# Eclectic-Sheep/sheeprl

Measured on NVIDIA H100. Metric: Dreamer-V3 train-steps/sec (S, bs16 seq64 horizon15, 64x64x3 obs), higher is better.
Workload: dtype f32

## Files before the change

sheeprl_b200/csrc/gemm_tc.cu:

```cuda
#include <cuda.h>
#include <cudaTypedefs.h>

#include <mutex>
#include <unordered_map>

#include "common.cuh"

namespace {

constexpr int BM = 128, BK = 32;
constexpr int NTHREADS = 384;
constexpr int NSPLIT_THREADS = 96;
constexpr int NCONS_WARPS = 8;
constexpr int PRODUCER_REGS = 56, CONSUMER_REGS = 224;
template <int BN> constexpr int stages_for() { return BN == 128 ? 3 : 5; }

__device__ __forceinline__ uint32_t smem_u32(const void* p) { return (uint32_t)__cvta_generic_to_shared(p); }

__device__ __forceinline__ void mbar_init(uint64_t* bar, uint32_t count) {
  asm volatile("mbarrier.init.shared::cta.b64 [%0], %1;" ::"r"(smem_u32(bar)), "r"(count) : "memory");
}
__device__ __forceinline__ void mbar_expect_tx(uint64_t* bar, uint32_t bytes) {
  asm volatile("mbarrier.arrive.expect_tx.shared::cta.b64 _, [%0], %1;" ::"r"(smem_u32(bar)), "r"(bytes) : "memory");
}
// ... 577 lines not shown
      c[j] = r;
    }
  }
}

#define LAUNCH_GEMM_TC(BN_, PASSES_, grid_, st_, ...)                                                                \
  do {                                                                                                               \
    const size_t smem__ = sizeof(Smem<BN_>) + 1024;                                                                  \
    RL_CUDA(cudaFuncSetAttribute(gemm_tc_kernel<BN_, PASSES_>, cudaFuncAttributeMaxDynamicSharedMemorySize, (int)smem__)); \
    gemm_tc_kernel<BN_, PASSES_><<<grid_, NTHREADS, smem__, st_>>>(__VA_ARGS__);                                      \
  } while (0)
#define DISPATCH_GEMM_TC(BN_val, passes_val, grid_, st_, ...)                                  \
  do {                                                                                          \
    if ((BN_val) == 64) {                                                                       \
      if ((passes_val) == 3) LAUNCH_GEMM_TC(64, 3, grid_, st_, __VA_ARGS__);                    \
      else LAUNCH_GEMM_TC(64, 1, grid_, st_, __VA_ARGS__);                                      \
    } else {                                                                                    \
      if ((passes_val) == 3) LAUNCH_GEMM_TC(128, 3, grid_, st_, __VA_ARGS__);                   \
      else LAUNCH_GEMM_TC(128, 1, grid_, st_, __VA_ARGS__);                                     \
    }                                                                                           \
  } while (0)

int launch_conv(int mode, const float* img, const float* Wp, float* out, const float* bias, int NB, int h, int w, int Cin,
                int Cout, cudaStream_t st) {
  TileGeo g = {};
  g.mode = mode; g.h = h; g.w = w; g.NB = NB; g.chunks = Cin / BK; g.Cout = Cout; g.ksplits = 1;
  g.passes = g_passes;
  RL_CHECK_ARG(conv_tile(h, w, NB, &g.bw, &g.bh, &g.bn), "image grid not tileable by 128 pixels");
  g.tiles_x = w / g.bw; g.tiles_y = h / g.bh;
  if (mode == MODE_UP && conv_up_merged(Cout)) mode = g.mode = MODE_UP4;
  const int taps = mode == MODE_DOWN ? 16 : (mode == MODE_UP4 ? 9 : 4);
  const int K = taps * Cin;
  CUtensorMap ma, mb;
  if (mode == MODE_DOWN) { if (int rc = get_map4(img, Cin, 2 * w, 2 * h, NB, g.bw, g.bh, g.bn, 2, &ma)) return rc; }
  else                   { if (int rc = get_map4(img, Cin, w, h, NB, g.bw, g.bh, g.bn, 1, &ma)) return rc; }
  const int BN = (mode == MODE_UP4) ? 128 : ((Cout <= 64) ? 64 : 128);
  const int brows = (mode == MODE_UP || mode == MODE_UP4) ? 4 * Cout : Cout;
  if (int rc = get_map(Wp, brows, K, K, BN, &mb)) return rc;
  const int mtiles = g.tiles_x * g.tiles_y * (NB / g.bn);
  g.mtiles = mtiles;
  g.ntiles = (mode == MODE_UP4) ? 1 : (Cout + BN - 1) / BN;
  dim3 grid(1, 1, mode == MODE_UP ? 4 : 1);
  grid.y = persistent_grid_y(mtiles * g.ntiles, grid.z);
  const int M = NB * h * w;
  DISPATCH_GEMM_TC(BN, g.passes, grid, st, ma, mb, out, bias, M, Cout, K, Cout, 0, g);
  RL_CHECK_LAUNCH();
  return B200RL_OK;
}

}

extern "C" int b200rl_set_matmul_precision(int tf32_passes) {
  RL_CHECK_ARG(tf32_passes == 1 || tf32_passes == 3, "tf32_passes must be 3 (fp32-accurate 3xTF32) or 1 (single TF32 pass)");
  g_passes = tf32_passes;
  return B200RL_OK;
}
extern "C" int b200rl_get_matmul_precision(void) { return g_passes; }

extern "C" long long b200rl_conv_pack_floats(int mode_up, int Cs, int Cb) {
  return (mode_up && conv_up_merged(Cb) ? 36LL : 16LL) * Cs * Cb;
}
extern "C" int b200rl_conv_tc_supported(int mode_up, int NB, int h, int w, int Cs, int Cb) {
  int bw, bh, bn;
  if (!conv_tile(h, w, NB, &bw, &bh, &bn)) return 0;
  const int Cin = mode_up ? Cs : Cb, Cout = mode_up ? Cb : Cs;
  if (Cin % BK != 0 || Cout < 16 || Cout % 4 != 0) return 0;
  return 1;
}
extern "C" int b200rl_conv_pack(const float* W, float* Wpacked, int mode_up, int Cs, int Cb, cudaStream_t st) {
  RL_CHECK_ARG(W && Wpacked, "null pointer");
  const long long n = (long long)Cs * Cb * 16;
  if (mode_up && conv_up_merged(Cb)) conv_pack_up4_kernel<<<ceil_div(36LL * Cs * Cb, 256), 256, 0, st>>>(W, Wpacked, Cs, Cb);
  else if (mode_up) conv_pack_up_kernel<<<ceil_div(n, 256), 256, 0, st>>>(W, Wpacked, Cs, Cb);
  else conv_pack_down_kernel<<<ceil_div(n, 256), 256, 0, st>>>(W, Wpacked, Cs, Cb);
  RL_CHECK_LAUNCH();
  return B200RL_OK;
}
extern "C" int b200rl_conv_down_tc(const float* big, const float* Wpacked, float* small_, int NB, int h, int w, int Cs,
                                   int Cb, cudaStream_t st) {
  RL_CHECK_ARG(big && Wpacked && small_, "null pointer");
  RL_CHECK_ARG(b200rl_conv_tc_supported(0, NB, h, w, Cs, Cb), "shape not eligible for the tensor-core conv path");
  return launch_conv(MODE_DOWN, big, Wpacked, small_, nullptr, NB, h, w, Cb, Cs, st);
}
extern "C" int b200rl_conv_up_tc(const float* small_, const float* Wpacked, float* big, const float* bias, int NB, int h,
                                 int w, int Cs, int Cb, cudaStream_t st) {
  RL_CHECK_ARG(big && Wpacked && small_, "null pointer");
  RL_CHECK_ARG(b200rl_conv_tc_supported(1, NB, h, w, Cs, Cb), "shape not eligible for the tensor-core conv path");
  return launch_conv(MODE_UP, small_, Wpacked, big, bias, NB, h, w, Cs, Cb, st);
}

extern "C" int b200rl_gemm_tc_supported(const float* A, const float* B, int M, int N, int K, int lda, int ldb,
                                        int transA, int transB) {
  (void)transA; (void)transB;
  if (M < 32 || N < 48 || K < 32) return 0;
  if ((lda & 3) || (ldb & 3)) return 0;
  if ((reinterpret_cast<uintptr_t>(A) & 15) || (reinterpret_cast<uintptr_t>(B) & 15)) return 0;
  return 1;
}

namespace {
struct FusedTail { float* part; int ks, mpad, ldw; };

int gemm_tc_impl(const float* A, const float* B, float* C, const float* bias, int M, int N, int K, int lda,
                 int ldb, int ldc, int transA, int transB, int accumulate, cudaStream_t st, FusedTail* fused) {
  RL_CHECK_ARG(A && B && (C || fused), "null pointer");
  RL_CHECK_ARG(b200rl_gemm_tc_supported(A, B, M, N, K, lda, ldb, transA, transB), "shape not eligible for the tensor-core path");
  const int BN = (N <= 64) ? 64 : 128;
  CUtensorMap ma, mb;
  if (!transA) { if (int rc = get_map(A, M, K, lda, BM, &ma)) return rc; }
  else         { if (int rc = get_map(A, K, M, lda, 32, &ma)) return rc; }
  if (transB)  { if (int rc = get_map(B, N, K, ldb, BN, &mb)) return rc; }
  else         { if (int rc = get_map(B, K, N, ldb, 32, &mb)) return rc; }
  dim3 grid((N + BN - 1) / BN, (M + BM - 1) / BM);
  TileGeo g = {};
  g.mode = MODE_GEMM;
  g.a_mn = transA ? 1 : 0;
  g.b_mn = transB ? 0 : 1;
  g.ksplits = 1;
  g.passes = g_passes;
  const int tiles = grid.x * grid.y, nkb = (K + BK - 1) / BK;
  if (tiles < 2 * kNumSMs && nkb >= 8) {
    int best = 1;
    float best_t = 1e30f;
    const int max_sp = nkb / 4 < 32 ? nkb / 4 : 32;
    for (int sp = 1; sp <= (max_sp < 1 ? 1 : max_sp); ++sp) {
      const int per = (nkb + sp - 1) / sp, real = (nkb + per - 1) / per;
      const int waves = (tiles * real + kNumSMs - 1) / kNumSMs;
      const float t = waves * (per * 0.8f + 4.0f) + (real > 1 ? 3.0f + 0.3f * real : 0.0f);
      if (t < best_t - 1e-3f) { best_t = t; best = real; }
    }
    g.ksplits = best;
  }
  if (g.ksplits > 1 || fused) {
    grid.z = g.ksplits;
    g.mpad = (int)grid.y * BM;
    g.ldw = (int)grid.x * BN;
    if (int rc = split_workspace((size_t)g.ksplits * g.mpad * g.ldw, st, &g.part)) return rc;
    if (fused) { g.force_part = 1; *fused = FusedTail{g.part, g.ksplits, g.mpad, g.ldw}; }
  }
  g.mtiles = (int)grid.y;
  g.ntiles = (int)grid.x;
  grid.x = 1;
  grid.y = persistent_grid_y(g.mtiles * g.ntiles, grid.z);
  DISPATCH_GEMM_TC(BN, g.passes, grid, st, ma, mb, C, bias, M, N, K, ldc, accumulate, g);
  RL_CHECK_LAUNCH();
  if (g.ksplits > 1 && !fused) {
    splitk_reduce_kernel<<<ceil_div((long long)M * ((N + 3) / 4), 256), 256, 0, st>>>(g.part, C, bias, M, N, ldc, g.ksplits, g.mpad,
                                                                                      g.ldw, accumulate);
    RL_CHECK_LAUNCH();
  }
  return B200RL_OK;
}

template <int NV>
__global__ void __launch_bounds__(256)
splitk_ln_kernel(const float* __restrict__ part, int ks, int mpad, int ldw, int M, int N, const float* __restrict__ gamma,
                 const float* __restrict__ beta, float eps, int act, float* __restrict__ pre, long long ldpre,
                 float* __restrict__ ln_out, long long ldln, int mode, const float* __restrict__ h_prev, long long ldh,
                 float* __restrict__ h_out, long long ldho, float* __restrict__ h_out2, long long ldho2) {
  const int lane = threadIdx.x & 31;
  const long long row = ((long long)blockIdx.x * blockDim.x + threadIdx.x) >> 5;
  if (row >= M) return;
  const int n4 = N >> 2;
  float4 v[NV];
#pragma unroll
  for (int i = 0; i < NV; ++i) v[i] = make_float4(0.f, 0.f, 0.f, 0.f);
#pragma unroll 4
  for (int z = 0; z < ks; ++z) {
    const float4* p = reinterpret_cast<const float4*>(part + ((size_t)z * mpad + row) * ldw);
#pragma unroll
    for (int i = 0; i < NV; ++i) {
      const int c = lane + 32 * i;
      if (c < n4) { const float4 t = __ldcg(p + c); v[i].x += t.x; v[i].y += t.y; v[i].z += t.z; v[i].w += t.w; }
    }
  }
  float s = 0.f;
#pragma unroll
  for (int i = 0; i < NV; ++i) {
    const int c = lane + 32 * i;
    if (c < n4) {
      if (pre) reinterpret_cast<float4*>(pre + row * ldpre)[c] = v[i];
      s += (v[i].x + v[i].y) + (v[i].z + v[i].w);
    }
  }
  const float mu = warp_sum(s) / (float)N;
  float q = 0.f;
#pragma unroll
  for (int i = 0; i < NV; ++i) {
    const int c = lane + 32 * i;
    if (c < n4) {
      const float dx = v[i].x - mu, dy = v[i].y - mu, dz = v[i].z - mu, dw = v[i].w - mu;
      q += (dx * dx + dy * dy) + (dz * dz + dw * dw);
    }
  }
  const float rstd = rsqrtf(warp_sum(q) / (float)N + eps);
#pragma unroll
  for (int i = 0; i < NV; ++i) {
    const int c = lane + 32 * i;
    if (c < n4) {
      const float4 g = reinterpret_cast<const float4*>(gamma)[c], b = reinterpret_cast<const float4*>(beta)[c];
      v[i].x = (v[i].x - mu) * rstd * g.x + b.x; v[i].y = (v[i].y - mu) * rstd * g.y + b.y;
      v[i].z = (v[i].z - mu) * rstd * g.z + b.z; v[i].w = (v[i].w - mu) * rstd * g.w + b.w;
      if (mode == 0 && act == 1) {
        v[i].x = v[i].x / (1.f + expf(-v[i].x)); v[i].y = v[i].y / (1.f + expf(-v[i].y));
        v[i].z = v[i].z / (1.f + expf(-v[i].z)); v[i].w = v[i].w / (1.f + expf(-v[i].w));
      }
      if (ln_out) reinterpret_cast<float4*>(ln_out + row * ldln)[c] = v[i];
    }
  }
  if (mode == 1) {
    constexpr int NR = NV / 3;
#pragma unroll
    for (int i = 0; i < NR; ++i) {
      const int c = lane + 32 * i;
      const float4 hp = reinterpret_cast<const float4*>(h_prev + row * ldh)[c];
      const float4 gr = v[i], gc = v[i + NR], gu = v[i + 2 * NR];
      float4 h;
      auto gate = [](float r_, float c_, float u_, float hprev) {
        const float r = 1.f / (1.f + expf(-r_));
        const float cand = tanhf(r * c_);
        const float u = 1.f / (1.f + expf(-(u_ - 1.f)));
        return u * cand + (1.f - u) * hprev;
      };
      h.x = gate(gr.x, gc.x, gu.x, hp.x); h.y = gate(gr.y, gc.y, gu.y, hp.y);
      h.z = gate(gr.z, gc.z, gu.z, hp.z); h.w = gate(gr.w, gc.w, gu.w, hp.w);
      reinterpret_cast<float4*>(h_out + row * ldho)[c] = h;
      if (h_out2) reinterpret_cast<float4*>(h_out2 + row * ldho2)[c] = h;
    }
  }
}
}

extern "C" int b200rl_gemm_tc(const float* A, const float* B, float* C, const float* bias, int M, int N, int K, int lda,
                              int ldb, int ldc, int transA, int transB, int accumulate, cudaStream_t st) {
  return gemm_tc_impl(A, B, C, bias, M, N, K, lda, ldb, ldc, transA, transB, accumulate, st, nullptr);
}

extern "C" int b200rl_gemm_ln_supported(const float* A, const float* B, int M, int N, int K, int lda, int ldb, int mode) {
  if (!b200rl_gemm_tc_supported(A, B, M, N, K, lda, ldb, 0, 1)) return 0;
  if (N % 4 || N > 1536) return 0;
  if (mode == 1 && (N % 384 != 0)) return 0;
  return 1;
}

extern "C" int b200rl_gemm_ln(const float* A, const float* W, int M, int N, int K, int lda, int ldw_, const float* gamma,
                              const float* beta, float eps, int act, float* pre, long long ldpre, float* out, long long ldout,
                              int mode, const float* h_prev, long long ldh, float* h_out, long long ldho, float* h_out2,
                              long long ldho2, cudaStream_t st) {
  RL_CHECK_ARG(A && W && gamma && beta, "null pointer");
  RL_CHECK_ARG(b200rl_gemm_ln_supported(A, W, M, N, K, lda, ldw_, mode), "shape not eligible for the fused product + LayerNorm");
  RL_CHECK_ARG(mode == 0 ? out != nullptr : (h_prev && h_out), "missing output");
  RL_CHECK_ARG(((reinterpret_cast<uintptr_t>(gamma) | reinterpret_cast<uintptr_t>(beta) | reinterpret_cast<uintptr_t>(pre) |
                 reinterpret_cast<uintptr_t>(out) | reinterpret_cast<uintptr_t>(h_prev) | reinterpret_cast<uintptr_t>(h_out) |
                 reinterpret_cast<uintptr_t>(h_out2)) & 15) == 0 &&
                   ((ldpre | ldout | ldh | ldho | ldho2) & 3) == 0,
               "fused product + LayerNorm needs 16-byte aligned rows");
  FusedTail ft;
  if (int rc = gemm_tc_impl(A, W, nullptr, nullptr, M, N, K, lda, ldw_, N, 0, 1, 0, st, &ft)) return rc;
  const int blocks = ceil_div((long long)M * 32, 256);
#define LAUNCH_SPLITK_LN(NV_)                                                                                              \
  splitk_ln_kernel<NV_><<<blocks, 256, 0, st>>>(ft.part, ft.ks, ft.mpad, ft.ldw, M, N, gamma, beta, eps, act, pre, ldpre, out, \
                                                ldout, mode, h_prev, ldh, h_out, ldho, h_out2, ldho2)
  if (mode == 1) {
    if (N == 384) LAUNCH_SPLITK_LN(3); else if (N == 768) LAUNCH_SPLITK_LN(6); else if (N == 1152) LAUNCH_SPLITK_LN(9);
    else LAUNCH_SPLITK_LN(12);
  } else if (N <= 128) LAUNCH_SPLITK_LN(1);
  else if (N <= 256) LAUNCH_SPLITK_LN(2);
  else if (N <= 512) LAUNCH_SPLITK_LN(4);
  else if (N <= 1024) LAUNCH_SPLITK_LN(8);
  else LAUNCH_SPLITK_LN(12);
#undef LAUNCH_SPLITK_LN
  RL_CHECK_LAUNCH();
  return B200RL_OK;
}

extern "C" int b200rl_conv_wgrad_mn_supported(int NB, int h, int w, int Cs, int Cb) {
  if (w <= 0 || h <= 0 || (w & (w - 1)) || (h & (h - 1))) return 0;
  const long long P = (long long)NB * h * w;
  if (Cb % 32 || Cs < 48 || Cs % 4 || P % 32 || P < 1024 || P > 2000000000LL) return 0;
  const int bw = w < 32 ? w : 32, bh = (32 / bw) < h ? (32 / bw) : h, bn = 32 / (bw * bh);
  return (bw * bh * bn == 32) && (NB % bn == 0);
}

extern "C" int b200rl_conv_wgrad_mn(const float* small_, const float* big, float* G, int NB, int h, int w, int Cs, int Cb,
                                    cudaStream_t st) {
  RL_CHECK_ARG(small_ && big && G, "null pointer");
  RL_CHECK_ARG(b200rl_conv_wgrad_mn_supported(NB, h, w, Cs, Cb), "shape not eligible for the in-place wgrad path");
  const int P = NB * h * w, M = 16 * Cb, N = Cs;
  TileGeo g = {};
  g.mode = MODE_GEMM; g.a_mn = 1; g.b_mn = 1; g.wg = 1; g.passes = g_passes;
  g.h = h; g.w = w; g.NB = NB; g.Cout = Cb;
  g.bw = w < 32 ? w : 32; g.bh = (32 / g.bw) < h ? (32 / g.bw) : h; g.bn = 32 / (g.bw * g.bh);
  CUtensorMap ma, mb;
  if (int rc = get_map4(big, Cb, 2 * w, 2 * h, NB, g.bw, g.bh, g.bn, 2, &ma)) return rc;
  if (int rc = get_map(small_, P, Cs, Cs, 32, &mb)) return rc;
  const int BN = (N <= 64) ? 64 : 128;
  dim3 grid((N + BN - 1) / BN, M / BM);
  const int tiles = grid.x * grid.y, nkb = P / BK;
  int sp = (2 * kNumSMs + tiles - 1) / tiles;
  if (sp > nkb / 8) sp = nkb / 8;
  if (sp < 1) sp = 1;
  const int per = (nkb + sp - 1) / sp;
  g.ksplits = (nkb + per - 1) / per;
  grid.z = g.ksplits;
  g.mtiles = (int)grid.y;
  g.ntiles = (int)grid.x;
  if (g.ksplits > 1) {
    g.mpad = (int)grid.y * BM;
    g.ldw = (int)grid.x * BN;
    if (int rc = split_workspace((size_t)g.ksplits * g.mpad * g.ldw, st, &g.part)) return rc;
  }
  grid.x = 1;
  grid.y = (unsigned)(g.mtiles * g.ntiles);
  DISPATCH_GEMM_TC(BN, g.passes, grid, st, ma, mb, G, nullptr, M, N, P, N, 0, g);
  RL_CHECK_LAUNCH();
  if (g.ksplits > 1) {
    splitk_reduce_kernel<<<ceil_div((long long)M * ((N + 3) / 4), 256), 256, 0, st>>>(g.part, G, nullptr, M, N, N, g.ksplits, g.mpad,
                                                                                      g.ldw, 0);
    RL_CHECK_LAUNCH();
  }
  return B200RL_OK;
}
```

sheeprl_b200/csrc/rssm.cu:

```cuda
#include "common.cuh"

namespace {

__global__ void gru_gate_fwd_kernel(const float* __restrict__ G, const float* __restrict__ Hin, float* __restrict__ Hout,
                                    long long M, int R, long long ldg, long long ldhi, long long ldho) {
  const long long idx = (long long)blockIdx.x * blockDim.x + threadIdx.x;
  if (idx >= M * R) return;
  const long long m = idx / R;
  const int j = (int)(idx - m * R);
  const float* g = G + m * ldg;
  const float r = sigmoidf_(g[j]);
  const float c = tanhf(r * g[R + j]);
  const float u = sigmoidf_(g[2 * R + j] - 1.f);
  const float h = Hin[m * ldhi + j];
  Hout[m * ldho + j] = u * c + (1.f - u) * h;
}

__global__ void gru_gate_bwd_kernel(const float* __restrict__ G, const float* __restrict__ Hin,
                                    const float* __restrict__ dH, float* __restrict__ dG, float* __restrict__ dHin,
                                    long long M, int R, long long ldg, long long ldhi, long long lddh,
                                    long long lddg, long long lddhi) {
  const long long idx = (long long)blockIdx.x * blockDim.x + threadIdx.x;
  if (idx >= M * R) return;
  const long long m = idx / R;
  const int j = (int)(idx - m * R);
  const float* g = G + m * ldg;
  const float gc = g[R + j];
  const float r = sigmoidf_(g[j]);
  const float c = tanhf(r * gc);
  const float u = sigmoidf_(g[2 * R + j] - 1.f);
  const float h = Hin[m * ldhi + j];
  const float dh = dH[m * lddh + j];
  const float du = dh * (c - h);
  const float drc = dh * u * (1.f - c * c);
  float* dg = dG + m * lddg;
  dg[j] = drc * gc * r * (1.f - r);
  dg[R + j] = drc * r;
  dg[2 * R + j] = du * u * (1.f - u);
  dHin[m * lddhi + j] = dh * (1.f - u);
}

__global__ void mask_mix_kernel(const float* __restrict__ prev, const float* __restrict__ init,
                                const float* __restrict__ first, float* __restrict__ out, long long M, int C,
                                long long ldp, long long ldo) {
  const long long idx = (long long)blockIdx.x * blockDim.x + threadIdx.x;
  if (idx >= M * C) return;
  const long long m = idx / C;
  const int c = (int)(idx - m * C);
  const float f = first[m];
  float v = (1.f - f) * prev[m * ldp + c];
  if (init) v += f * init[c];
  out[m * ldo + c] = v;
}

__global__ void mask_bwd_kernel(const float* __restrict__ dIn, const float* __restrict__ first,
                                float* __restrict__ dPrev, float* __restrict__ dInit, int M, int C, long long ldi,
                                long long ldp) {
  const int c = blockIdx.x * blockDim.x + threadIdx.x;
  if (c >= C) return;
  float s = 0.f;
  for (int m = 0; m < M; ++m) {
    const float f = first[m];
    const float d = dIn[m * ldi + c];
    dPrev[m * ldp + c] = (1.f - f) * d;
    s = fmaf(f, d, s);
  }
  if (dInit) dInit[c] += s;
}

struct GroupStats {
  float raw_max, raw_sum;
  float lse;
};

__device__ __forceinline__ float unimix_logprob(float s, float unimix, float invK, float& pm) {
  pm = (1.f - unimix) * s + unimix * invK;
  return logf(fminf(fmaxf(pm, kFp32Eps), 1.f - kFp32Eps));
}

__device__ __forceinline__ GroupStats group_stats(const float* x, int K, float unimix, int lane) {
  GroupStats st;
  float mx = -INFINITY;
  for (int c = lane; c < K; c += 32) mx = fmaxf(mx, x[c]);
  mx = warp_max(mx);
  float sm = 0.f;
  for (int c = lane; c < K; c += 32) sm += expf(x[c] - mx);
  sm = warp_sum(sm);
  st.raw_max = mx;
  st.raw_sum = sm;
  const float invK = 1.f / (float)K;
  float lmx = -INFINITY;
  for (int c = lane; c < K; c += 32) {
    float l = x[c];
    if (unimix > 0.f) { float pm; l = unimix_logprob(expf(x[c] - mx) / sm, unimix, invK, pm); }
    lmx = fmaxf(lmx, l);
  }
  lmx = warp_max(lmx);
  float ls = 0.f;
  for (int c = lane; c < K; c += 32) {
    float l = x[c];
    if (unimix > 0.f) { float pm; l = unimix_logprob(expf(x[c] - mx) / sm, unimix, invK, pm); }
    ls += expf(l - lmx);
  }
  ls = warp_sum(ls);
  st.lse = lmx + logf(ls);
  return st;
}

__global__ void __launch_bounds__(256)
cat_sample_kernel(const float* __restrict__ raw, const float* __restrict__ noise, float* __restrict__ onehot,
                  float* __restrict__ mix_out, long long M, int groups, int K, long long ldr, long long ldn,
                  long long ldo, long long ldm, float unimix) {
  const int lane = threadIdx.x & 31;
  const long long warp = ((long long)blockIdx.x * blockDim.x + threadIdx.x) >> 5;
  if (warp >= M * groups) return;
  const long long m = warp / groups;
  const int g = (int)(warp - m * groups);
  const float* x = raw + m * ldr + (long long)g * K;
  const GroupStats st = group_stats(x, K, unimix, lane);
  const float invK = 1.f / (float)K;
  float lgmax = -INFINITY;
  for (int c = lane; c < K; c += 32) {
    float l = x[c];
    if (unimix > 0.f) { float pm; l = unimix_logprob(expf(x[c] - st.raw_max) / st.raw_sum, unimix, invK, pm); }
    if (mix_out) mix_out[m * ldm + (long long)g * K + c] = l;
    lgmax = fmaxf(lgmax, l - st.lse);
  }
  lgmax = warp_max(lgmax);
  float psum = 0.f;
  for (int c = lane; c < K; c += 32) {
    float l = x[c];
    if (unimix > 0.f) { float pm; l = unimix_logprob(expf(x[c] - st.raw_max) / st.raw_sum, unimix, invK, pm); }
    psum += expf(l - st.lse - lgmax);
  }
  psum = warp_sum(psum);
  if (!onehot) return;
  float best = -INFINITY;
  int besti = 0x7fffffff;
  for (int c = lane; c < K; c += 32) {
    float l = x[c];
    if (unimix > 0.f) { float pm; l = unimix_logprob(expf(x[c] - st.raw_max) / st.raw_sum, unimix, invK, pm); }
    float p = expf(l - st.lse - lgmax) / psum;
    if (noise) p = p / noise[m * ldn + (long long)g * K + c];
    if (p > best) { best = p; besti = c; }
  }
#pragma unroll
  for (int o = 16; o > 0; o >>= 1) {
    const float ob = __shfl_xor_sync(0xffffffffu, best, o);
    const int oi = __shfl_xor_sync(0xffffffffu, besti, o);
    if (ob > best || (ob == best && oi < besti)) { best = ob; besti = oi; }
  }
  for (int c = lane; c < K; c += 32) onehot[m * ldo + (long long)g * K + c] = (c == besti) ? 1.f : 0.f;
}

__device__ __forceinline__ void cat_sample_lane(float xv, bool on, int K, int lane, float unimix,
                                                const float* __restrict__ noise_row, float* __restrict__ onehot_row,
                                                float* __restrict__ mix_row) {
  const float mx = warp_max(xv);
  const float sm = warp_sum(on ? expf(xv - mx) : 0.f);
  const float invK = 1.f / (float)K;
  float l = xv;
  if (unimix > 0.f && on) { float pm; l = unimix_logprob(expf(xv - mx) / sm, unimix, invK, pm); }
  const float lmx = warp_max(on ? l : -INFINITY);
  const float ls = warp_sum(on ? expf(l - lmx) : 0.f);
  const float lse = lmx + logf(ls);
  if (mix_row && on) mix_row[lane] = l;
  const float lgmax = warp_max(on ? l - lse : -INFINITY);
  const float e = on ? expf(l - lse - lgmax) : 0.f;
  const float psum = warp_sum(e);
  if (!onehot_row) return;
  float best = -INFINITY;
  int besti = 0x7fffffff;
  if (on) {
    float p = e / psum;
    if (noise_row) p = p / noise_row[lane];
    if (p > best) { best = p; besti = lane; }
  }
#pragma unroll
  for (int o = 16; o > 0; o >>= 1) {
    const float ob = __shfl_xor_sync(0xffffffffu, best, o);
    const int oi = __shfl_xor_sync(0xffffffffu, besti, o);
    if (ob > best || (ob == best && oi < besti)) { best = ob; besti = oi; }
  }
  if (on) onehot_row[lane] = (lane == besti) ? 1.f : 0.f;
}

__global__ void __launch_bounds__(256)
cat_sample_small_kernel(const float* __restrict__ raw, const float* __restrict__ noise, float* __restrict__ onehot,
                        float* __restrict__ mix_out, long long M, int groups, int K, long long ldr, long long ldn,
                        long long ldo, long long ldm, float unimix) {
  const int lane = threadIdx.x & 31;
  const long long warp = ((long long)blockIdx.x * blockDim.x + threadIdx.x) >> 5;
  if (warp >= M * groups) return;
  const long long m = warp / groups;
  const int g = (int)(warp - m * groups);
  const bool on = lane < K;
  const float xv = on ? raw[m * ldr + (long long)g * K + lane] : -INFINITY;
  cat_sample_lane(xv, on, K, lane, unimix, noise ? noise + m * ldn + (long long)g * K : nullptr,
                  onehot ? onehot + m * ldo + (long long)g * K : nullptr, mix_out ? mix_out + m * ldm + (long long)g * K : nullptr);
}

__global__ void __launch_bounds__(256)
head_sample_kernel(const float* __restrict__ X, const float* __restrict__ W, const float* __restrict__ bias,
                   const float* __restrict__ noise, float* __restrict__ raw, float* __restrict__ onehot, long long M, int Kin,
                   int A, long long ldx, long long ldw, long long ldr, long long ldn, long long ldo, float unimix) {
  const int lane = threadIdx.x & 31;
  const long long m = ((long long)blockIdx.x * blockDim.x + threadIdx.x) >> 5;
  if (m >= M) return;
  const int k4 = Kin >> 2;
  float4 x[8];
#pragma unroll
  for (int i = 0; i < 8; ++i) {
    const int c = lane + 32 * i;
    x[i] = c < k4 ? reinterpret_cast<const float4*>(X + m * ldx)[c] : make_float4(0.f, 0.f, 0.f, 0.f);
  }
  float mine = -INFINITY;
  for (int a = 0; a < A; ++a) {
    const float4* w = reinterpret_cast<const float4*>(W + (long long)a * ldw);
    float acc = 0.f;
#pragma unroll
    for (int i = 0; i < 8; ++i) {
      const int c = lane + 32 * i;
      if (c < k4) {
        const float4 t = __ldg(w + c);
        acc = fmaf(x[i].x, t.x, acc); acc = fmaf(x[i].y, t.y, acc); acc = fmaf(x[i].z, t.z, acc); acc = fmaf(x[i].w, t.w, acc);
      }
    }
    acc = warp_sum(acc);
    if (lane == a) mine = acc + (bias ? bias[a] : 0.f);
  }
  const bool on = lane < A;
  if (on) raw[m * ldr + lane] = mine;
  cat_sample_lane(mine, on, A, lane, unimix, noise ? noise + m * ldn : nullptr, onehot + m * ldo, nullptr);
}

__global__ void __launch_bounds__(256)
cat_sample_bwd_kernel(const float* __restrict__ raw, const float* __restrict__ dz, const float* __restrict__ dmix,
                      float* __restrict__ draw, long long M, int groups, int K, long long ldr, long long lddz,
                      long long lddm, long long lddr, float unimix) {
  const int lane = threadIdx.x & 31;
  const long long warp = ((long long)blockIdx.x * blockDim.x + threadIdx.x) >> 5;
  if (warp >= M * groups) return;
  const long long m = warp / groups;
  const int g = (int)(warp - m * groups);
  const long long go = (long long)g * K;
  const float* x = raw + m * ldr + go;
  const GroupStats st = group_stats(x, K, unimix, lane);
  const float invK = 1.f / (float)K;
  float pdz = 0.f;
  if (dz) {
    for (int c = lane; c < K; c += 32) {
      float l = x[c];
      if (unimix > 0.f) { float pm; l = unimix_logprob(expf(x[c] - st.raw_max) / st.raw_sum, unimix, invK, pm); }
      pdz = fmaf(expf(l - st.lse), dz[m * lddz + go + c], pdz);
    }
    pdz = warp_sum(pdz);
  }
  float sds = 0.f;
  for (int c = lane; c < K; c += 32) {
    const float s = expf(x[c] - st.raw_max) / st.raw_sum;
    float pm = 0.f, l = x[c];
    if (unimix > 0.f) l = unimix_logprob(s, unimix, invK, pm);
    float gg = dmix ? dmix[m * lddm + go + c] : 0.f;
    if (dz) gg += expf(l - st.lse) * (dz[m * lddz + go + c] - pdz);
    if (unimix > 0.f) {
      const bool inside = pm >= kFp32Eps && pm <= 1.f - kFp32Eps;
      const float ds = inside ? gg * (1.f - unimix) / pm : 0.f;
      sds = fmaf(s, ds, sds);
    }
  }
  sds = warp_sum(sds);
  for (int c = lane; c < K; c += 32) {
    const float s = expf(x[c] - st.raw_max) / st.raw_sum;
    float pm = 0.f, l = x[c];
    if (unimix > 0.f) l = unimix_logprob(s, unimix, invK, pm);
    float gg = dmix ? dmix[m * lddm + go + c] : 0.f;
    if (dz) gg += expf(l - st.lse) * (dz[m * lddz + go + c] - pdz);
    if (unimix > 0.f) {
      const bool inside = pm >= kFp32Eps && pm <= 1.f - kFp32Eps;
      const float ds = inside ? gg * (1.f - unimix) / pm : 0.f;
      gg = s * (ds - sds);
    }
    draw[m * lddr + go + c] = gg;
  }
}

__global__ void __launch_bounds__(256)
kl_loss_grad_kernel(const float* __restrict__ post, const float* __restrict__ prior, float* __restrict__ d_post,
                    float* __restrict__ d_prior, float* __restrict__ rows, int groups, int K, long long ldp,
                    long long ldq, long long lddp, long long lddq, float kl_dyn, float kl_rep, float free_nats,
                    float coef ) {
  __shared__ float red[32];
  const long long m = blockIdx.x;
  const int lane = threadIdx.x & 31, wid = threadIdx.x >> 5, nw = blockDim.x >> 5;
  const float* lp0 = post + m * ldp;
  const float* lq0 = prior + m * ldq;
  float kl = 0.f, hp = 0.f, hq = 0.f;
  for (int g = wid; g < groups; g += nw) {
    const float* a = lp0 + (long long)g * K;
    const float* b = lq0 + (long long)g * K;
    float ma = -INFINITY, mb = -INFINITY;
    for (int c = lane; c < K; c += 32) { ma = fmaxf(ma, a[c]); mb = fmaxf(mb, b[c]); }
    ma = warp_max(ma); mb = warp_max(mb);
    float sa = 0.f, sb = 0.f;
    for (int c = lane; c < K; c += 32) { sa += expf(a[c] - ma); sb += expf(b[c] - mb); }
    const float lsea = ma + logf(warp_sum(sa)), lseb = mb + logf(warp_sum(sb));
    float t = 0.f, ea = 0.f, eb = 0.f;
    for (int c = lane; c < K; c += 32) {
      const float lpa = a[c] - lsea, lqb = b[c] - lseb;
      const float pa = expf(lpa), pb = expf(lqb);
      t = fmaf(pa, lpa - lqb, t);
      ea = fmaf(-pa, lpa, ea);
      eb = fmaf(-pb, lqb, eb);
    }
    kl += t; hp += ea; hq += eb;
  }
  kl = block_sum(kl, red);
  hp = block_sum(hp, red);
  hq = block_sum(hq, red);
  if (threadIdx.x == 0) {
    rows[m * 4 + 0] = kl;
    rows[m * 4 + 1] = (kl_dyn + kl_rep) * fmaxf(kl, free_nats);
    rows[m * 4 + 2] = hp;
    rows[m * 4 + 3] = hq;
  }
  const float live = (kl > free_nats) ? coef : 0.f;
  for (int g = wid; g < groups; g += nw) {
    const float* a = lp0 + (long long)g * K;
    const float* b = lq0 + (long long)g * K;
    float ma = -INFINITY, mb = -INFINITY;
    for (int c = lane; c < K; c += 32) { ma = fmaxf(ma, a[c]); mb = fmaxf(mb, b[c]); }
    ma = warp_max(ma); mb = warp_max(mb);
    float sa = 0.f, sb = 0.f;
    for (int c = lane; c < K; c += 32) { sa += expf(a[c] - ma); sb += expf(b[c] - mb); }
    const float lsea = ma + logf(warp_sum(sa)), lseb = mb + logf(warp_sum(sb));
    float t = 0.f;
    for (int c = lane; c < K; c += 32) {
      const float lpa = a[c] - lsea, lqb = b[c] - lseb;
      t = fmaf(expf(lpa), lpa - lqb, t);
    }
    const float klg = warp_sum(t);
    for (int c = lane; c < K; c += 32) {
      const float lpa = a[c] - lsea, lqb = b[c] - lseb;
      const float pa = expf(lpa), pb = expf(lqb);
      d_prior[m * lddq + (long long)g * K + c] = kl_dyn * live * (pb - pa);
      d_post[m * lddp + (long long)g * K + c] = kl_rep * live * pa * ((lpa - lqb) - klg);
    }
  }
}


__global__ void __launch_bounds__(256)
onehot_linear_kernel(const float* __restrict__ z, const float* __restrict__ act, const float* __restrict__ WT,
                     float* __restrict__ out, int S, int K, int A, int N, long long ldz, long long lda, long long ldo,
                     const float* __restrict__ gamma, const float* __restrict__ beta, float eps, float* __restrict__ pre,
                     long long ldpre) {
  __shared__ int idx[64];
  __shared__ float av[32];
  __shared__ float red[8];
  const long long m = blockIdx.x;
  const int lane = threadIdx.x & 31, warp = threadIdx.x >> 5;
  for (int g = warp; g < S; g += (int)(blockDim.x >> 5)) {
    int found = 0;
    for (int c0 = 0; c0 < K; c0 += 32) {
      const int c = c0 + lane;
      const unsigned b = __ballot_sync(0xffffffffu, c < K && z[m * ldz + (long long)g * K + c] != 0.f);
      if (b) { found = c0 + __ffs(b) - 1; break; }
    }
    if (lane == 0) idx[g] = found;
  }
  if (threadIdx.x < A) av[threadIdx.x] = act[m * lda + threadIdx.x];
  __syncthreads();
  if (gamma == nullptr) {
    for (int n = threadIdx.x; n < N; n += blockDim.x) {
      float acc = 0.f;
#pragma unroll 8
      for (int g = 0; g < S; ++g) acc += __ldg(WT + ((long long)g * K + idx[g]) * N + n);
      for (int a = 0; a < A; ++a) acc = fmaf(av[a], __ldg(WT + ((long long)S * K + a) * N + n), acc);
      out[m * ldo + n] = acc;
    }
    return;
  }
  const int t = threadIdx.x, nw = (blockDim.x + 31) >> 5;
  const float4* W4 = reinterpret_cast<const float4*>(WT);
  const int n4 = N >> 2;
  float4 acc = make_float4(0.f, 0.f, 0.f, 0.f);
#pragma unroll 8
  for (int g = 0; g < S; ++g) {
    const float4 w = __ldg(W4 + ((long long)g * K + idx[g]) * n4 + t);
    acc.x += w.x; acc.y += w.y; acc.z += w.z; acc.w += w.w;
  }
  for (int a = 0; a < A; ++a) {
    const float4 w = __ldg(W4 + ((long long)S * K + a) * n4 + t);
    acc.x = fmaf(av[a], w.x, acc.x); acc.y = fmaf(av[a], w.y, acc.y); acc.z = fmaf(av[a], w.z, acc.z); acc.w = fmaf(av[a], w.w, acc.w);
  }
  if (pre) *reinterpret_cast<float4*>(pre + m * ldpre + 4 * t) = acc;
  auto block_sum = [&](float x) {
    x = warp_sum(x);
    __syncthreads();
    if (lane == 0) red[warp] = x;
    __syncthreads();
    float r = 0.f;
    for (int w = 0; w < nw; ++w) r += red[w];
    return r;
  };
  const float mu = block_sum((acc.x + acc.y) + (acc.z + acc.w)) / (float)N;
  const float dx = acc.x - mu, dy = acc.y - mu, dz = acc.z - mu, dw = acc.w - mu;
  const float rstd = rsqrtf(block_sum((dx * dx + dy * dy) + (dz * dz + dw * dw)) / (float)N + eps);
  const float4 gm = reinterpret_cast<const float4*>(gamma)[t], bt = reinterpret_cast<const float4*>(beta)[t];
  float4 y;
  y.x = dx * rstd * gm.x + bt.x; y.y = dy * rstd * gm.y + bt.y; y.z = dz * rstd * gm.z + bt.z; y.w = dw * rstd * gm.w + bt.w;
  y.x = y.x / (1.f + expf(-y.x)); y.y = y.y / (1.f + expf(-y.y)); y.z = y.z / (1.f + expf(-y.z)); y.w = y.w / (1.f + expf(-y.w));
  *reinterpret_cast<float4*>(out + m * ldo + 4 * t) = y;
}

}

extern "C" int b200rl_gru_gate_fwd(const float* G, const float* Hin, float* Hout, long long M, int R, long long ldg,
                                   long long ldhi, long long ldho, cudaStream_t st) {
  RL_CHECK_ARG(G && Hin && Hout, "null pointer");
  if (M * R <= 0) return B200RL_OK;
  gru_gate_fwd_kernel<<<ceil_div(M * R, 256), 256, 0, st>>>(G, Hin, Hout, M, R, ldg, ldhi, ldho);
  RL_CHECK_LAUNCH();
  return B200RL_OK;
}

extern "C" int b200rl_gru_gate_bwd(const float* G, const float* Hin, const float* dH, float* dG, float* dHin,
                                   long long M, int R, long long ldg, long long ldhi, long long lddh, long long lddg,
                                   long long lddhi, cudaStream_t st) {
  RL_CHECK_ARG(G && Hin && dH && dG && dHin, "null pointer");
  if (M * R <= 0) return B200RL_OK;
  gru_gate_bwd_kernel<<<ceil_div(M * R, 256), 256, 0, st>>>(G, Hin, dH, dG, dHin, M, R, ldg, ldhi, lddh, lddg, lddhi);
  RL_CHECK_LAUNCH();
  return B200RL_OK;
}

extern "C" int b200rl_mask_mix(const float* prev, const float* init, const float* first, float* out, long long M,
                               int C, long long ldp, long long ldo, cudaStream_t st) {
  RL_CHECK_ARG(prev && first && out, "null pointer");
  if (M * C <= 0) return B200RL_OK;
  mask_mix_kernel<<<ceil_div(M * C, 256), 256, 0, st>>>(prev, init, first, out, M, C, ldp, ldo);
  RL_CHECK_LAUNCH();
  return B200RL_OK;
}

extern "C" int b200rl_mask_bwd(const float* dIn, const float* first, float* dPrev, float* dInit, int M, int C,
                               long long ldi, long long ldp, cudaStream_t st) {
  RL_CHECK_ARG(dIn && first && dPrev, "null pointer");
  if (M <= 0 || C <= 0) return B200RL_OK;
  mask_bwd_kernel<<<ceil_div(C, 128), 128, 0, st>>>(dIn, first, dPrev, dInit, M, C, ldi, ldp);
  RL_CHECK_LAUNCH();
  return B200RL_OK;
}

extern "C" int b200rl_cat_sample(const float* raw, const float* noise, float* onehot, float* mix_out, long long M,
                                 int groups, int K, long long ldr, long long ldn, long long ldo, long long ldm,
                                 float unimix, cudaStream_t st) {
  RL_CHECK_ARG(raw, "null pointer");
  RL_CHECK_ARG(groups > 0 && K > 0, "bad groups / classes");
  if (M <= 0) return B200RL_OK;
  const long long warps = M * groups;
  if (K <= 32)
    cat_sample_small_kernel<<<ceil_div(warps, 8), 256, 0, st>>>(raw, noise, onehot, mix_out, M, groups, K, ldr, ldn, ldo,
                                                                ldm, unimix);
  else
    cat_sample_kernel<<<ceil_div(warps, 8), 256, 0, st>>>(raw, noise, onehot, mix_out, M, groups, K, ldr, ldn, ldo, ldm,
                                                          unimix);
  RL_CHECK_LAUNCH();
  return B200RL_OK;
}

extern "C" int b200rl_head_sample_supported(const float* X, const float* W, int Kin, int A, long long ldx, long long ldw) {
  return A > 0 && A <= 32 && Kin > 0 && Kin <= 1024 && Kin % 4 == 0 && ldx % 4 == 0 && ldw % 4 == 0 &&
         ((reinterpret_cast<uintptr_t>(X) | reinterpret_cast<uintptr_t>(W)) & 15) == 0;
}

extern "C" int b200rl_head_sample(const float* X, const float* W, const float* bias, const float* noise, float* raw,
                                  float* onehot, long long M, int Kin, int A, long long ldx, long long ldw, long long ldr,
                                  long long ldn, long long ldo, float unimix, cudaStream_t st) {
  RL_CHECK_ARG(X && W && raw && onehot, "null pointer");
  RL_CHECK_ARG(b200rl_head_sample_supported(X, W, Kin, A, ldx, ldw),
               "head_sample: A <= 32, Kin <= 1024, 16-byte aligned rows");
  if (M <= 0) return B200RL_OK;
  head_sample_kernel<<<ceil_div(M * 32, 256), 256, 0, st>>>(X, W, bias, noise, raw, onehot, M, Kin, A, ldx, ldw, ldr, ldn, ldo,
                                                            unimix);
  RL_CHECK_LAUNCH();
  return B200RL_OK;
}

extern "C" int b200rl_cat_sample_bwd(const float* raw, const float* dz, const float* dmix, float* draw, long long M,
                                     int groups, int K, long long ldr, long long lddz, long long lddm,
                                     long long lddr, float unimix, cudaStream_t st) {
  RL_CHECK_ARG(raw && draw, "null pointer");
  RL_CHECK_ARG(groups > 0 && K > 0, "bad groups / classes");
  if (M <= 0) return B200RL_OK;
  const long long warps = M * groups;
  cat_sample_bwd_kernel<<<ceil_div(warps, 8), 256, 0, st>>>(raw, dz, dmix, draw, M, groups, K, ldr, lddz, lddm, lddr,
                                                            unimix);
  RL_CHECK_LAUNCH();
  return B200RL_OK;
}

extern "C" int b200rl_kl_loss_grad(const float* post_mix, const float* prior_mix, float* d_post, float* d_prior,
                                   float* rows, long long M, int groups, int K, long long ldp, long long ldq,
                                   long long lddp, long long lddq, float kl_dyn, float kl_rep, float free_nats,
                                   float regularizer, float scale, cudaStream_t st) {
  RL_CHECK_ARG(post_mix && prior_mix && d_post && d_prior && rows, "null pointer");
  if (M <= 0) return B200RL_OK;
  kl_loss_grad_kernel<<<(unsigned)M, 256, 0, st>>>(post_mix, prior_mix, d_post, d_prior, rows, groups, K, ldp, ldq,
                                                   lddp, lddq, kl_dyn, kl_rep, free_nats, scale * regularizer);
  RL_CHECK_LAUNCH();
  return B200RL_OK;
}

extern "C" int b200rl_onehot_linear_supported(int S, int K, int A, int N) {
  return S > 0 && S <= 64 && K > 0 && A >= 0 && A <= 32 && N > 0;
}

extern "C" int b200rl_onehot_linear_ln_supported(const float* WT, const float* gamma, const float* beta, const float* out,
                                                 const float* pre, int N, long long ldo, long long ldpre) {
  return N >= 128 && N <= 1024 && N % 128 == 0 && ldo % 4 == 0 && ldpre % 4 == 0 &&
         ((reinterpret_cast<uintptr_t>(WT) | reinterpret_cast<uintptr_t>(gamma) | reinterpret_cast<uintptr_t>(beta) |
           reinterpret_cast<uintptr_t>(out) | reinterpret_cast<uintptr_t>(pre)) & 15) == 0;
}

extern "C" int b200rl_onehot_linear(const float* z, const float* act, const float* WT, float* out, long long M, int S,
                                    int K, int A, int N, long long ldz, long long lda, long long ldo, cudaStream_t st) {
  RL_CHECK_ARG(z && act && WT && out, "null pointer");
  RL_CHECK_ARG(b200rl_onehot_linear_supported(S, K, A, N), "bad dims (S <= 64 groups, A <= 32)");
  if (M <= 0) return B200RL_OK;
  onehot_linear_kernel<<<(unsigned)M, 256, 0, st>>>(z, act, WT, out, S, K, A, N, ldz, lda, ldo, nullptr, nullptr, 0.f, nullptr, 0);
  RL_CHECK_LAUNCH();
  return B200RL_OK;
}

extern "C" int b200rl_onehot_linear_ln(const float* z, const float* act, const float* WT, const float* gamma,
                                       const float* beta, float eps, float* pre, long long ldpre, float* out, long long M,
                                       int S, int K, int A, int N, long long ldz, long long lda, long long ldo,
                                       cudaStream_t st) {
  RL_CHECK_ARG(z && act && WT && out && gamma && beta, "null pointer");
  RL_CHECK_ARG(b200rl_onehot_linear_supported(S, K, A, N), "bad dims (S <= 64 groups, A <= 32)");
  RL_CHECK_ARG(b200rl_onehot_linear_ln_supported(WT, gamma, beta, out, pre, N, ldo, ldpre),
               "onehot_linear_ln: N a multiple of 128 up to 1024, 16-byte aligned rows");
  if (M <= 0) return B200RL_OK;
  onehot_linear_kernel<<<(unsigned)M, N / 4, 0, st>>>(z, act, WT, out, S, K, A, N, ldz, lda, ldo, gamma, beta, eps, pre, ldpre);
  RL_CHECK_LAUNCH();
  return B200RL_OK;
}
```

Baseline: 58.01.

## Prefetch LN params early, 8-lane categorical sampling, batched one-hot index scan

```diff
diff --git a/sheeprl_b200/csrc/gemm_tc.cu b/sheeprl_b200/csrc/gemm_tc.cu
--- a/sheeprl_b200/csrc/gemm_tc.cu
+++ b/sheeprl_b200/csrc/gemm_tc.cu
@@ -753,7 +753,7 @@
   return B200RL_OK;
 }
 
-template <int NV>
+template <int NV, bool EARLY>
 __global__ void __launch_bounds__(256)
 splitk_ln_kernel(const float* __restrict__ part, int ks, int mpad, int ldw, int M, int N, const float* __restrict__ gamma,
                  const float* __restrict__ beta, float eps, int act, float* __restrict__ pre, long long ldpre,
@@ -763,6 +763,19 @@
   const long long row = ((long long)blockIdx.x * blockDim.x + threadIdx.x) >> 5;
   if (row >= M) return;
   const int n4 = N >> 2;
+  constexpr int NR = NV / 3;
+  float4 gv[EARLY ? NV : 1], bv[EARLY ? NV : 1], hp[EARLY && NR > 0 ? NR : 1];
+  if constexpr (EARLY) {
+#pragma unroll
+    for (int i = 0; i < NV; ++i) {
+      const int c = lane + 32 * i;
+      if (c < n4) { gv[i] = reinterpret_cast<const float4*>(gamma)[c]; bv[i] = reinterpret_cast<const float4*>(beta)[c]; }
+    }
+    if (mode == 1) {
+#pragma unroll
+      for (int i = 0; i < NR; ++i) hp[i] = reinterpret_cast<const float4*>(h_prev + row * ldh)[lane + 32 * i];
+    }
+  }
   float4 v[NV];
 #pragma unroll
   for (int i = 0; i < NV; ++i) v[i] = make_float4(0.f, 0.f, 0.f, 0.f);
@@ -799,7 +812,9 @@
   for (int i = 0; i < NV; ++i) {
     const int c = lane + 32 * i;
     if (c < n4) {
-      const float4 g = reinterpret_cast<const float4*>(gamma)[c], b = reinterpret_cast<const float4*>(beta)[c];
+      float4 g, b;
+      if constexpr (EARLY) { g = gv[i]; b = bv[i]; }
+      else { g = reinterpret_cast<const float4*>(gamma)[c]; b = reinterpret_cast<const float4*>(beta)[c]; }
       v[i].x = (v[i].x - mu) * rstd * g.x + b.x; v[i].y = (v[i].y - mu) * rstd * g.y + b.y;
       v[i].z = (v[i].z - mu) * rstd * g.z + b.z; v[i].w = (v[i].w - mu) * rstd * g.w + b.w;
       if (mode == 0 && act == 1) {
@@ -810,11 +825,12 @@
     }
   }
   if (mode == 1) {
-    constexpr int NR = NV / 3;
 #pragma unroll
     for (int i = 0; i < NR; ++i) {
       const int c = lane + 32 * i;
-      const float4 hp = reinterpret_cast<const float4*>(h_prev + row * ldh)[c];
+      float4 hpv;
+      if constexpr (EARLY) hpv = hp[i];
+      else hpv = reinterpret_cast<const float4*>(h_prev + row * ldh)[c];
       const float4 gr = v[i], gc = v[i + NR], gu = v[i + 2 * NR];
       float4 h;
       auto gate = [](float r_, float c_, float u_, float hprev) {
@@ -823,8 +839,8 @@
         const float u = 1.f / (1.f + expf(-(u_ - 1.f)));
         return u * cand + (1.f - u) * hprev;
       };
-      h.x = gate(gr.x, gc.x, gu.x, hp.x); h.y = gate(gr.y, gc.y, gu.y, hp.y);
-      h.z = gate(gr.z, gc.z, gu.z, hp.z); h.w = gate(gr.w, gc.w, gu.w, hp.w);
+      h.x = gate(gr.x, gc.x, gu.x, hpv.x); h.y = gate(gr.y, gc.y, gu.y, hpv.y);
+      h.z = gate(gr.z, gc.z, gu.z, hpv.z); h.w = gate(gr.w, gc.w, gu.w, hpv.w);
       reinterpret_cast<float4*>(h_out + row * ldho)[c] = h;
       if (h_out2) reinterpret_cast<float4*>(h_out2 + row * ldho2)[c] = h;
     }
@@ -860,8 +876,14 @@
   if (int rc = gemm_tc_impl(A, W, nullptr, nullptr, M, N, K, lda, ldw_, N, 0, 1, 0, st, &ft)) return rc;
   const int blocks = ceil_div((long long)M * 32, 256);
 #define LAUNCH_SPLITK_LN(NV_)                                                                                              \
-  splitk_ln_kernel<NV_><<<blocks, 256, 0, st>>>(ft.part, ft.ks, ft.mpad, ft.ldw, M, N, gamma, beta, eps, act, pre, ldpre, out, \
-                                                ldout, mode, h_prev, ldh, h_out, ldho, h_out2, ldho2)
+  do {                                                                                                                     \
+    if (blocks <= kNumSMs)                                                                                                 \
+      splitk_ln_kernel<NV_, true><<<blocks, 256, 0, st>>>(ft.part, ft.ks, ft.mpad, ft.ldw, M, N, gamma, beta, eps, act, pre, \
+                                                          ldpre, out, ldout, mode, h_prev, ldh, h_out, ldho, h_out2, ldho2);   \
+    else                                                                                                                   \
+      splitk_ln_kernel<NV_, false><<<blocks, 256, 0, st>>>(ft.part, ft.ks, ft.mpad, ft.ldw, M, N, gamma, beta, eps, act, pre, \
+                                                           ldpre, out, ldout, mode, h_prev, ldh, h_out, ldho, h_out2, ldho2);  \
+  } while (0)
   if (mode == 1) {
     if (N == 384) LAUNCH_SPLITK_LN(3); else if (N == 768) LAUNCH_SPLITK_LN(6); else if (N == 1152) LAUNCH_SPLITK_LN(9);
     else LAUNCH_SPLITK_LN(12);
diff --git a/sheeprl_b200/csrc/rssm.cu b/sheeprl_b200/csrc/rssm.cu
--- a/sheeprl_b200/csrc/rssm.cu
+++ b/sheeprl_b200/csrc/rssm.cu
@@ -153,9 +153,8 @@
   for (int c = lane; c < K; c += 32) onehot[m * ldo + (long long)g * K + c] = (c == besti) ? 1.f : 0.f;
 }
 
-__device__ __forceinline__ void cat_sample_lane(float xv, bool on, int K, int lane, float unimix,
-                                                const float* __restrict__ noise_row, float* __restrict__ onehot_row,
-                                                float* __restrict__ mix_row) {
+__device__ __forceinline__ void cat_sample_lane(float xv, bool on, int K, int lane, float unimix, bool has_noise, float nv,
+                                                float* __restrict__ onehot_row, float* __restrict__ mix_row) {
   const float mx = warp_max(xv);
   const float sm = warp_sum(on ? expf(xv - mx) : 0.f);
   const float invK = 1.f / (float)K;
@@ -173,7 +172,7 @@
   int besti = 0x7fffffff;
   if (on) {
     float p = e / psum;
-    if (noise_row) p = p / noise_row[lane];
+    if (has_noise) p = p / nv;
     if (p > best) { best = p; besti = lane; }
   }
 #pragma unroll
@@ -185,19 +184,102 @@
   if (on) onehot_row[lane] = (lane == besti) ? 1.f : 0.f;
 }
 
+__device__ __forceinline__ float group8_max(const float (&v)[4]) {
+  float r = fmaxf(fmaxf(v[0], v[2]), fmaxf(v[1], v[3]));
+#pragma unroll
+  for (int o = 4; o > 0; o >>= 1) r = fmaxf(r, __shfl_xor_sync(0xffffffffu, r, o));
+  return r;
+}
+__device__ __forceinline__ float group8_sum(const float (&v)[4]) {
+  float r = (v[0] + v[2]) + (v[1] + v[3]);
+#pragma unroll
+  for (int o = 4; o > 0; o >>= 1) r += __shfl_xor_sync(0xffffffffu, r, o);
+  return r;
+}
+__device__ __forceinline__ void take_best(float& b, int& i, float ob, int oi) {
+  if (ob > b || (ob == b && oi < i)) { b = ob; i = oi; }
+}
+
 __global__ void __launch_bounds__(256)
 cat_sample_small_kernel(const float* __restrict__ raw, const float* __restrict__ noise, float* __restrict__ onehot,
                         float* __restrict__ mix_out, long long M, int groups, int K, long long ldr, long long ldn,
                         long long ldo, long long ldm, float unimix) {
-  const int lane = threadIdx.x & 31;
-  const long long warp = ((long long)blockIdx.x * blockDim.x + threadIdx.x) >> 5;
-  if (warp >= M * groups) return;
-  const long long m = warp / groups;
-  const int g = (int)(warp - m * groups);
-  const bool on = lane < K;
-  const float xv = on ? raw[m * ldr + (long long)g * K + lane] : -INFINITY;
-  cat_sample_lane(xv, on, K, lane, unimix, noise ? noise + m * ldn + (long long)g * K : nullptr,
-                  onehot ? onehot + m * ldo + (long long)g * K : nullptr, mix_out ? mix_out + m * ldm + (long long)g * K : nullptr);
+  const int sl = threadIdx.x & 7;
+  const long long gid = ((long long)blockIdx.x * blockDim.x + threadIdx.x) >> 3;
+  const bool live = gid < M * groups;
+  const long long m = live ? gid / groups : 0;
+  const int g = live ? (int)(gid - m * groups) : 0;
+  const long long ro = m * ldr + (long long)g * K;
+  float xv[4], nv[4];
+  bool on[4];
+#pragma unroll
+  for (int j = 0; j < 4; ++j) {
+    const int c = sl + 8 * j;
+    on[j] = live && c < K;
+    xv[j] = on[j] ? raw[ro + c] : -INFINITY;
+    nv[j] = (noise && onehot && on[j]) ? noise[m * ldn + (long long)g * K + c] : 1.f;
+  }
+  const float mx = group8_max(xv);
+  float t[4];
+#pragma unroll
+  for (int j = 0; j < 4; ++j) t[j] = on[j] ? expf(xv[j] - mx) : 0.f;
+  const float sm = group8_sum(t);
+  const float invK = 1.f / (float)K;
+  float l[4];
+#pragma unroll
+  for (int j = 0; j < 4; ++j) {
+    l[j] = xv[j];
+    if (unimix > 0.f && on[j]) { float pm; l[j] = unimix_logprob(t[j] / sm, unimix, invK, pm); }
+    t[j] = on[j] ? l[j] : -INFINITY;
+  }
+  const float lmx = group8_max(t);
+#pragma unroll
+  for (int j = 0; j < 4; ++j) t[j] = on[j] ? expf(l[j] - lmx) : 0.f;
+  const float lse = lmx + logf(group8_sum(t));
+#pragma unroll
+  for (int j = 0; j < 4; ++j) {
+    if (mix_out && on[j]) mix_out[m * ldm + (long long)g * K + sl + 8 * j] = l[j];
+    t[j] = on[j] ? l[j] - lse : -INFINITY;
+  }
+  const float lgmax = group8_max(t);
+  float e[4];
+#pragma unroll
+  for (int j = 0; j < 4; ++j) e[j] = on[j] ? expf(l[j] - lse - lgmax) : 0.f;
+  const float psum = group8_sum(e);
+  if (!onehot) return;
+  float best[4];
+  int besti[4];
+#pragma unroll
+  for (int j = 0; j < 4; ++j) {
+    best[j] = -INFINITY;
+    besti[j] = 0x7fffffff;
+    if (on[j]) {
+      float p = e[j] / psum;
+      if (noise) p = p / nv[j];
+      if (p > best[j]) { best[j] = p; besti[j] = sl + 8 * j; }
+    }
+  }
+#pragma unroll
+  for (int h = 2; h > 0; h >>= 1) {
+    float b[4];
+    int bi[4];
+#pragma unroll
+    for (int j = 0; j < 4; ++j) { b[j] = best[j]; bi[j] = besti[j]; take_best(b[j], bi[j], best[j ^ h], besti[j ^ h]); }
+#pragma unroll
+    for (int j = 0; j < 4; ++j) { best[j] = b[j]; besti[j] = bi[j]; }
+  }
+#pragma unroll
+  for (int o = 4; o > 0; o >>= 1)
+#pragma unroll
+    for (int j = 0; j < 4; ++j) {
+      const float ob = __shfl_xor_sync(0xffffffffu, best[j], o);
+      const int oi = __shfl_xor_sync(0xffffffffu, besti[j], o);
+      take_best(best[j], besti[j], ob, oi);
+    }
+  const long long oo = m * ldo + (long long)g * K;
+#pragma unroll
+  for (int j = 0; j < 4; ++j)
+    if (on[j]) onehot[oo + sl + 8 * j] = (sl + 8 * j == besti[j]) ? 1.f : 0.f;
 }
 
 __global__ void __launch_bounds__(256)
@@ -208,6 +290,8 @@
   const long long m = ((long long)blockIdx.x * blockDim.x + threadIdx.x) >> 5;
   if (m >= M) return;
   const int k4 = Kin >> 2;
+  const bool on = lane < A;
+  const float nv = (noise && on) ? noise[m * ldn + lane] : 1.f;
   float4 x[8];
 #pragma unroll
   for (int i = 0; i < 8; ++i) {
@@ -229,9 +313,8 @@
     acc = warp_sum(acc);
     if (lane == a) mine = acc + (bias ? bias[a] : 0.f);
   }
-  const bool on = lane < A;
   if (on) raw[m * ldr + lane] = mine;
-  cat_sample_lane(mine, on, A, lane, unimix, noise ? noise + m * ldn : nullptr, onehot + m * ldo, nullptr);
+  cat_sample_lane(mine, on, A, lane, unimix, noise != nullptr, nv, onehot + m * ldo, nullptr);
 }
 
 __global__ void __launch_bounds__(256)
@@ -359,15 +442,36 @@
   __shared__ float av[32];
   __shared__ float red[8];
   const long long m = blockIdx.x;
-  const int lane = threadIdx.x & 31, warp = threadIdx.x >> 5;
-  for (int g = warp; g < S; g += (int)(blockDim.x >> 5)) {
-    int found = 0;
-    for (int c0 = 0; c0 < K; c0 += 32) {
-      const int c = c0 + lane;
-      const unsigned b = __ballot_sync(0xffffffffu, c < K && z[m * ldz + (long long)g * K + c] != 0.f);
-      if (b) { found = c0 + __ffs(b) - 1; break; }
-    }
-    if (lane == 0) idx[g] = found;
+  const int lane = threadIdx.x & 31, warp = threadIdx.x >> 5, nwarps = (int)(blockDim.x >> 5);
+  const int t = threadIdx.x;
+  float4 gm = make_float4(0.f, 0.f, 0.f, 0.f), bt = gm;
+  if (gamma) { gm = reinterpret_cast<const float4*>(gamma)[t]; bt = reinterpret_cast<const float4*>(beta)[t]; }
+  if (K <= 32) {
+    for (int g0 = warp; g0 < S; g0 += 8 * nwarps) {
+      float v[8];
+#pragma unroll
+      for (int j = 0; j < 8; ++j) {
+        const int g = g0 + j * nwarps;
+        v[j] = (g < S && lane < K) ? z[m * ldz + (long long)g * K + lane] : 0.f;
+      }
+#pragma unroll
+      for (int j = 0; j < 8; ++j) {
+        const int g = g0 + j * nwarps;
+        if (g >= S) break;
+        const unsigned b = __ballot_sync(0xffffffffu, v[j] != 0.f);
+        if (lane == 0) idx[g] = b ? __ffs(b) - 1 : 0;
+      }
+    }
+  } else {
+    for (int g = warp; g < S; g += nwarps) {
+      int found = 0;
+      for (int c0 = 0; c0 < K; c0 += 32) {
+        const int c = c0 + lane;
+        const unsigned b = __ballot_sync(0xffffffffu, c < K && z[m * ldz + (long long)g * K + c] != 0.f);
+        if (b) { found = c0 + __ffs(b) - 1; break; }
+      }
+      if (lane == 0) idx[g] = found;
+    }
   }
   if (threadIdx.x < A) av[threadIdx.x] = act[m * lda + threadIdx.x];
   __syncthreads();
@@ -381,7 +485,7 @@
     }
     return;
   }
-  const int t = threadIdx.x, nw = (blockDim.x + 31) >> 5;
+  const int nw = (blockDim.x + 31) >> 5;
   const float4* W4 = reinterpret_cast<const float4*>(WT);
   const int n4 = N >> 2;
   float4 acc = make_float4(0.f, 0.f, 0.f, 0.f);
@@ -407,7 +511,6 @@
   const float mu = block_sum((acc.x + acc.y) + (acc.z + acc.w)) / (float)N;
   const float dx = acc.x - mu, dy = acc.y - mu, dz = acc.z - mu, dw = acc.w - mu;
   const float rstd = rsqrtf(block_sum((dx * dx + dy * dy) + (dz * dz + dw * dw)) / (float)N + eps);
-  const float4 gm = reinterpret_cast<const float4*>(gamma)[t], bt = reinterpret_cast<const float4*>(beta)[t];
   float4 y;
   y.x = dx * rstd * gm.x + bt.x; y.y = dy * rstd * gm.y + bt.y; y.z = dz * rstd * gm.z + bt.z; y.w = dw * rstd * gm.w + bt.w;
   y.x = y.x / (1.f + expf(-y.x)); y.y = y.y / (1.f + expf(-y.y)); y.z = y.z / (1.f + expf(-y.z)); y.w = y.w / (1.f + expf(-y.w));
@@ -461,7 +564,7 @@
   if (M <= 0) return B200RL_OK;
   const long long warps = M * groups;
   if (K <= 32)
-    cat_sample_small_kernel<<<ceil_div(warps, 8), 256, 0, st>>>(raw, noise, onehot, mix_out, M, groups, K, ldr, ldn, ldo,
+    cat_sample_small_kernel<<<ceil_div(warps, 32), 256, 0, st>>>(raw, noise, onehot, mix_out, M, groups, K, ldr, ldn, ldo,
                                                                 ldm, unimix);
   else
     cat_sample_kernel<<<ceil_div(warps, 8), 256, 0, st>>>(raw, noise, onehot, mix_out, M, groups, K, ldr, ldn, ldo, ldm,
```

After: 58.86 (median of 6 runs). 1.01x the previous value.
